# DakeQQ/Audio-Denoiser-ONNX

Measured on AMD Instinct MI355X. Metric: audio_seconds_per_second (GTCRN 16 kHz, batch=256 x 1 s chunks; RTF = 1/value), higher is better.
Workload: dtype f32; 1 GPU; GTCRN 16 kHz, batch=256 x 1 s chunks, fp32, int16 PCM in/out resident in HBM (BASELINE.json configs[1]); chunks_per_gpu=256, chunks_total=256, ranks=1, chunk_samples=16000, out_samples=15872, weights=seeded reference-architecture GTCRN (tests/golden/gtcrn_seed0.adew), stitch_all_gather=False

## Files before the change

### audio_denoiser_onnx_amd/csrc/ade_device.h

```cpp
#pragma once

#include "ade_internal.h"

namespace ade {
namespace dev {

__device__ __forceinline__ float fast_rcp(float x) { return __builtin_amdgcn_rcpf(x); }
__device__ __forceinline__ float fast_sqrt(float x) { return __builtin_amdgcn_sqrtf(x); }
__device__ __forceinline__ float fast_rsq(float x) { return __builtin_amdgcn_rsqf(x); }
__device__ __forceinline__ float sigmoid_f(float x) { return fast_rcp(1.0f + __expf(-x)); }
__device__ __forceinline__ float tanh_f(float x) {
    return 1.0f - 2.0f * fast_rcp(__expf(2.0f * x) + 1.0f);
}
__device__ __forceinline__ float prelu_f(float x, float a) { return x >= 0.0f ? x : a * x; }
__device__ __forceinline__ double shfl_xor_f64(double v, int mask) {
    union { double d; int i[2]; } u;
    u.d = v;
    u.i[0] = __shfl_xor(u.i[0], mask, 64);
    u.i[1] = __shfl_xor(u.i[1], mask, 64);
    return u.d;
}
__device__ __forceinline__ float prelu_sel(float a) { return a <= 1.0f ? __builtin_inff() : -__builtin_inff(); }
__device__ __forceinline__ float prelu_m(float x, float ax, float sel) { return __builtin_amdgcn_fmed3f(x, ax, sel); }

// ... 98 lines not shown
#define ADE_OPAQUE_V(x) asm volatile("" : "+v"(x))
#else
#define ADE_OPAQUE_V(x) ((void)0)
#endif
template <class T>
__device__ __forceinline__ T cload(const void ADE_CONSTANT_AS* p) {
    static_assert(sizeof(T) % 4 == 0, "dword-sized structs only");
    union U { T v; unsigned w[sizeof(T) / 4]; __device__ U() {} } u;
    const unsigned ADE_CONSTANT_AS* s = (const unsigned ADE_CONSTANT_AS*)p;
#pragma unroll
    for (size_t i = 0; i < sizeof(T) / 4; ++i) u.w[i] = s[i];
    return u.v;
}
typedef const float ADE_CONSTANT_AS* cfptr;
__device__ __forceinline__ cfptr cptr(const float* p) { return (cfptr)p; }

__device__ __forceinline__ void wave_sync() { __builtin_amdgcn_wave_barrier(); }
__device__ __forceinline__ float2 fcmul(float2 a, float2 b) { return make_float2(a.x * b.x - a.y * b.y, a.x * b.y + a.y * b.x); }
__device__ __forceinline__ void fradix4(float2* v) {
    const float2 a0 = make_float2(v[0].x + v[2].x, v[0].y + v[2].y);
    const float2 a1 = make_float2(v[0].x - v[2].x, v[0].y - v[2].y);
    const float2 a2 = make_float2(v[1].x + v[3].x, v[1].y + v[3].y);
    const float2 d = make_float2(v[1].x - v[3].x, v[1].y - v[3].y);
    const float2 a3 = make_float2(d.y, -d.x);
    v[0] = make_float2(a0.x + a2.x, a0.y + a2.y);
    v[1] = make_float2(a1.x + a3.x, a1.y + a3.y);
    v[2] = make_float2(a0.x - a2.x, a0.y - a2.y);
    v[3] = make_float2(a1.x - a3.x, a1.y - a3.y);
}
__device__ __forceinline__ void fft256_inplace(float2* v, float2* buf, int lane, const float2* __restrict__ tw256) {
// ... 29 lines not shown
}

#if defined(__AMDGCN__)
typedef unsigned ade_v4u __attribute__((ext_vector_type(4)));
__device__ __forceinline__ float4 xld4(const float* base, int float_off) {
    const __amdgpu_buffer_rsrc_t r = __builtin_amdgcn_make_buffer_rsrc(const_cast<float*>(base), 0, 0x7fffffff, 0x00020000);
    const ade_v4u v = __builtin_amdgcn_raw_buffer_load_b128(r, float_off * 4, 0, 16);
    return make_float4(__int_as_float((int)v.x), __int_as_float((int)v.y), __int_as_float((int)v.z), __int_as_float((int)v.w));
}
__device__ __forceinline__ void xst4(float* base, int float_off, const float4& v) {
    const __amdgpu_buffer_rsrc_t r = __builtin_amdgcn_make_buffer_rsrc(base, 0, 0x7fffffff, 0x00020000);
    ade_v4u u;
    u.x = (unsigned)__float_as_int(v.x); u.y = (unsigned)__float_as_int(v.y); u.z = (unsigned)__float_as_int(v.z); u.w = (unsigned)__float_as_int(v.w);
    __builtin_amdgcn_raw_buffer_store_b128(u, r, float_off * 4, 0, 16);
}
__device__ __forceinline__ float xld1(const float* p) { return __hip_atomic_load(p, __ATOMIC_RELAXED, __HIP_MEMORY_SCOPE_AGENT); }
__device__ __forceinline__ void xst1(float* p, float v) { __hip_atomic_store(p, v, __ATOMIC_RELAXED, __HIP_MEMORY_SCOPE_AGENT); }
__device__ __forceinline__ unsigned xflag_load(const unsigned* p) { return __hip_atomic_load(p, __ATOMIC_RELAXED, __HIP_MEMORY_SCOPE_AGENT); }
__device__ __forceinline__ void xflag_store(unsigned* p, unsigned v) { __hip_atomic_store(p, v, __ATOMIC_RELAXED, __HIP_MEMORY_SCOPE_AGENT); }
__device__ __forceinline__ void xdrain() { asm volatile("s_waitcnt vmcnt(0)" ::: "memory"); }
#else
__device__ __forceinline__ float4 xld4(const float* base, int float_off) { return *reinterpret_cast<const float4*>(base + float_off); }
__device__ __forceinline__ void xst4(float* base, int float_off, const float4& v) { *reinterpret_cast<float4*>(base + float_off) = v; }
__device__ __forceinline__ float xld1(const float* p) { return *p; }
__device__ __forceinline__ void xst1(float* p, float v) { *p = v; }
__device__ __forceinline__ unsigned xflag_load(const unsigned* p) { return *(const volatile unsigned*)p; }
__device__ __forceinline__ void xflag_store(unsigned* p, unsigned v) { *(volatile unsigned*)p = v; }
__device__ __forceinline__ void xdrain() {}
#endif
#if defined(__AMDGCN__)
__device__ __forceinline__ int xlimit() {
    const int ADE_CONSTANT_AS* p = (const int ADE_CONSTANT_AS*)__builtin_amdgcn_kernarg_segment_ptr();
    asm volatile("" : "+s"(p));
    return *p;
}
#else
__device__ __forceinline__ int xlimit() { return 20000000; }
#endif
__device__ __forceinline__ int xcode(int flag_index) { return (int)((blockIdx.x + 1u) << 4) | flag_index; }
__device__ __forceinline__ void xwait(unsigned* flag, int* err, int code) {
    if (xflag_load(flag) == 0u) {
        const long long t0 = wall_clock64();
        const int limit = xlimit();
        bool looked = false;
        do {
            __builtin_amdgcn_s_sleep(4);
            const long long dt = wall_clock64() - t0;
            if (dt > (limit >> 4) && !looked) {
                looked = true;
                if (*reinterpret_cast<volatile int*>(err) != 0) return;
            }
            if (dt > limit) {
                volatile int* const e = reinterpret_cast<volatile int*>(err);
                if (*e == 0) *e = code;
                return;
            }
        } while (xflag_load(flag) == 0u);
    }
    xflag_store(flag, 0u);
}

#if defined(__AMDGCN__)
__device__ __forceinline__ unsigned sys_load(const unsigned* p) { return __hip_atomic_load(p, __ATOMIC_RELAXED, __HIP_MEMORY_SCOPE_SYSTEM); }
__device__ __forceinline__ void sys_store(unsigned* p, unsigned v) { __hip_atomic_store(p, v, __ATOMIC_RELAXED, __HIP_MEMORY_SCOPE_SYSTEM); }
__device__ __forceinline__ void sys_acquire() { __builtin_amdgcn_fence(__ATOMIC_ACQUIRE, ""); }
__device__ __forceinline__ void sys_release() { __builtin_amdgcn_fence(__ATOMIC_RELEASE, ""); asm volatile("s_waitcnt vmcnt(0)" ::: "memory"); }
#else
__device__ __forceinline__ unsigned sys_load(const unsigned* p) { return *(const volatile unsigned*)p; }
__device__ __forceinline__ void sys_store(unsigned* p, unsigned v) { *(volatile unsigned*)p = v; }
__device__ __forceinline__ void sys_acquire() {}
__device__ __forceinline__ void sys_release() {}
#endif
__device__ __forceinline__ void wait_rows_in(const unsigned* ready, unsigned epoch, int* err, int code) {
    if (sys_load(ready) != epoch) {
        const long long t0 = wall_clock64();
        const int limit = xlimit();
        do {
            __builtin_amdgcn_s_sleep(8);
            if (wall_clock64() - t0 > limit) {
                volatile int* const e = reinterpret_cast<volatile int*>(err);
                if (*e == 0) *e = code;
                break;
            }
        } while (sys_load(ready) != epoch);
    }
    sys_acquire();
}
__device__ __forceinline__ void signal_rows_out(unsigned* count, unsigned* done, unsigned epoch, unsigned wgs) {
    sys_release();
#if defined(__AMDGCN__)
    const unsigned old = __hip_atomic_fetch_add(count, 1u, __ATOMIC_RELAXED, __HIP_MEMORY_SCOPE_AGENT);
#else
    const unsigned old = (*count)++;
#endif
    if (old + 1u == wgs) {
        xflag_store(count, 0u);
        sys_store(done, epoch);
    }
}

__device__ __forceinline__ void set_prio(int p) {
    if (p == 0) __builtin_amdgcn_s_setprio(0);
    else if (p == 1) __builtin_amdgcn_s_setprio(1);
    else if (p == 2) __builtin_amdgcn_s_setprio(2);
    else __builtin_amdgcn_s_setprio(3);
}
// ... 6 lines not shown
```

### audio_denoiser_onnx_amd/csrc/ade_stage_frontback.h

```cpp
#pragma once
#include "ade_stage_net.h"

namespace ade {
namespace stage {

constexpr int kWbuf = 264;
constexpr size_t kTabFloats = 512 + 2 * 256 + 2 * 264;
constexpr int kBmCap = 16;
constexpr int kBsCap = 4;

__device__ __forceinline__ float2 rfft_bin(float2 zk, float2 zp, float2 w) {
    const float2 e = make_float2(0.5f * (zk.x + zp.x), 0.5f * (zk.y - zp.y));
    const float2 d = make_float2(0.5f * (zk.x - zp.x), 0.5f * (zk.y + zp.y));
    const float2 o = make_float2(d.y, -d.x);
    return make_float2(e.x + (w.x * o.x - w.y * o.y), e.y + (w.x * o.y + w.y * o.x));
}

struct LdsTabs { const float* win; const float2* tw256; const float2* tw512; };
template <class G>
__device__ __forceinline__ LdsTabs stage_tables(float* dst, const FftTabs& t, int tid) {
    constexpr int kFusedThreads = G::kThreads;
    float* win = dst;
    float* tw256 = dst + 512;
    float* tw512 = tw256 + 512;
    for (int i = tid; i < 512; i += kFusedThreads) { win[i] = t.win[i]; tw256[i] = reinterpret_cast<const float*>(t.tw256)[i]; }
    for (int i = tid; i < 514; i += kFusedThreads) tw512[i] = reinterpret_cast<const float*>(t.tw512)[i];
    return LdsTabs{win, reinterpret_cast<const float2*>(tw256), reinterpret_cast<const float2*>(tw512)};
}

__device__ __forceinline__ void load_frame_pairs(const int16_t* __restrict__ row, int L, int t, int lane, bool live, bool pair_ok, int* raw, int centre = kNfft / 2) {
#pragma unroll
    for (int r = 0; r < 4; ++r) {
        const int n = lane + 64 * r;
        const int j0 = kHop * t + 2 * n - centre;
        if (!live) {
            raw[r] = 0;
        } else if (pair_ok && j0 >= 0 && j0 + 1 < L) {
            raw[r] = *reinterpret_cast<const int*>(row + j0);
        } else {
            int ja = j0, jb = j0 + 1;
            ja = ja < 0 ? -ja : (ja >= L ? 2 * (L - 1) - ja : ja);
            jb = jb < 0 ? -jb : (jb >= L ? 2 * (L - 1) - jb : jb);
            raw[r] = ((int)row[ja] & 0xffff) | ((int)row[jb] << 16);
// ... 33 lines not shown
    static_assert(kFusedThreads == 1024 || kFusedThreads == 512 || kFusedThreads == 256, "front / back conv rounds: 64 lanes per frame");
    constexpr int kBmRows = G::kLean ? 0 : kBmCap;
    const int T = sg.T, tbeg = sg.t0, tend = sg.t0 + sg.nT;
    float2* wbuf_all = reinterpret_cast<float2*>(smem);
    float* feat = smem + kTileF * kWbuf * 2;
    float4* E0 = reinterpret_cast<float4*>(feat + kFrontFeatFloats);
    float* E0f = reinterpret_cast<float*>(E0);
    float* tabmem = reinterpret_cast<float*>(E0 + 4 * kTileP1);
    float* erbw = tabmem + kTabFloats;
    float* w0t = erbw + kBmRows * kErbBands;
    float* w1t = w0t + kC0TailW;
    int* red = reinterpret_cast<int*>(w1t + kC1TailW);
    int tid_ = threadIdx.x;
    ADE_OPAQUE_V(tid_);
    const int tid = tid_, wave = tid >> 6, lane = tid & 63;
    const int16_t* row = pcm + (size_t)chunk * L;
    const int P0 = T * kF1, P = T * kFw;
    float* e0c = e0 + (size_t)chunk * kCh * P0;
    float* e1c = e1 + (size_t)chunk * kCh * P;
    float* specc = spec + (size_t)chunk * T * 2 * kBinsPad;
    ADE_CLK(32);
    const bool pair_ok = ((L & 1) == 0) && ((reinterpret_cast<size_t>(row) & 3) == 0);
    int raw[4];
    const int centre = sg.stream ? 0 : kNfft / 2;
    load_frame_pairs(row, L, tbeg + wave, lane, tbeg + wave < tend, pair_ok, raw, centre);
    const LdsTabs lt = stage_tables<G>(tabmem, tabs, tid);
    const bool erb_lds = erb.count <= kBmRows;
    if (erb_lds)
        for (int i = tid; i < erb.count * kErbBands; i += kFusedThreads) erbw[i] = erb.w[i];
    const int erb_s0 = erb.start[lane];
    for (int i = tid; i < kC0TailW; i += kFusedThreads) w0t[i] = c0.w[i];
    for (int i = tid; i < kC1TailW; i += kFusedThreads) w1t[i] = c1.w[i];
    const float b0t = c0.b[tid & 15], b1t = c1.b[tid & 15];

    if (!dc_rows) {
        int s = 0;
        if (((L & 7) == 0) && ((reinterpret_cast<size_t>(row) & 15) == 0)) {
            constexpr int kMeanLoads = 2048 / kFusedThreads;
            const int4* r4 = reinterpret_cast<const int4*>(row);
            const int4* z4 = reinterpret_cast<const int4*>(g_zero4);
            const int n4 = L >> 3;
            for (int i0 = tid; i0 < n4; i0 += kMeanLoads * kFusedThreads) {
                int4 q[kMeanLoads];
#pragma unroll
                for (int u = 0; u < kMeanLoads; ++u) {
                    const int i = i0 + u * kFusedThreads;
                    q[u] = *(i < n4 ? r4 + i : z4);
                }
#pragma unroll
                for (int u = 0; u < kMeanLoads; ++u)
                    s += (int)(short)(q[u].x & 0xffff) + (q[u].x >> 16) + (int)(short)(q[u].y & 0xffff) + (q[u].y >> 16)
                       + (int)(short)(q[u].z & 0xffff) + (q[u].z >> 16) + (int)(short)(q[u].w & 0xffff) + (q[u].w >> 16);
            }
        } else {
            for (int i = tid; i < L; i += kFusedThreads) s += (int)row[i];
        }
#pragma unroll
        for (int off = 32; off >= 1; off >>= 1) s += __shfl_xor(s, off);
        if (lane == 0) red[wave] = s;
    }
    __syncthreads();
    float dc;
    if (dc_rows) {
        dc = dc_rows[chunk];
    } else {
        long long tot = 0;
#pragma unroll
        for (int i = 0; i < kTileF; ++i) tot += red[i];
        dc = (float)((double)tot / ((double)L * 32768.0));
    }
    ADE_CLK(33);
    long long clk_prev = ADE_CLK_START();
    const cfptr c0b = cptr(c0.b), c1b = cptr(c1.b);
    const cfptr c0e = cptr(c0.w) + 5 * 9 * 16;

    for (int t0 = tbeg; t0 < tend; t0 += kTileF) {
        const int nf = tend - t0 < kTileF ? tend - t0 : kTileF;
        {
            int tq = tid;
// ... 44 lines not shown
                float* fr = feat + (size_t)wave * 3 * kErb;
#pragma unroll
                for (int r = 0; r < 5; ++r) {
                    if (r == 4 && lane != 0) break;
                    const int k = r < 4 ? lane + 64 * r : 256;
                    const float2 x = buf[k];
                    specc[((size_t)t * 2 + 0) * kBinsPad + k] = x.x;
                    specc[((size_t)t * 2 + 1) * kBinsPad + k] = x.y;
                    if (k < kErbLow) {
                        fr[k] = fast_sqrt((x.x * x.x + x.y * x.y) + 1e-12f);
                        fr[kErb + k] = x.x;
                        fr[2 * kErb + k] = x.y;
                    }
                }
                if (erb_lds) erb_merge(erbw, erb.count, erb_s0, buf, lane, fr);
                else erb_merge(erb.w, erb.count, erb_s0, buf, lane, fr);
            }
        }
        __syncthreads();
        ADE_CLK(34);
        ADE_CLK_ACC(40);
        {
            int tq = tid;
            ADE_OPAQUE_V(tq);
            const int tl = tq >> 6, g = (tq >> 4) & 3, j = tq & 15;
            if (tl < nf) {
                const float* fr = feat + (size_t)tl * 3 * kErb;
                float wa[6];
#pragma unroll
                for (int kk = 0; kk < 6; ++kk) wa[kk] = c0e[((kk >> 1) * 8 + 4 * (kk & 1) + g) * 16 + j];
                v4f cb;
// ... 124 lines not shown
    constexpr int kGroupShift = (kFusedThreads == 1024 ? 9 : (kFusedThreads == 512 ? 8 : 7));
    constexpr bool kLean = G::kLean;
    const int T = sg.T, tbeg = sg.t0, tend = sg.t0 + sg.nT;
    float4* S = reinterpret_cast<float4*>(smem);
    float* Sf = smem;
    float2* wbuf_all = reinterpret_cast<float2*>(smem);
    float4* D = S + 4 * kTileP;
    float* Df = reinterpret_cast<float*>(D);
    float* M = reinterpret_cast<float*>(D + 4 * kTileP1);
    float* acc = Df;
    float* cbuf = M + kTileF * 2 * kErbPad;
    float* tabmem = cbuf + kHop;
    float* bsw = tabmem + kTabFloats;
    float* w3t = bsw + kBsCap * kErbHigh;
    float* w4t = w3t + kC3TailW;
    float* wsum = kLean ? const_cast<float*>(tabs.win_sum) : w4t + kC4TailW;
    int* bss = reinterpret_cast<int*>(wsum + kHop);
    float* pend = kLean ? sg.xo + kXPendOff : reinterpret_cast<float*>(bss + kErbHigh);
    int tid_ = threadIdx.x;
    ADE_OPAQUE_V(tid_);
    const int tid = tid_;
    const int P0 = T * kF1, P = T * kFw;
    const float* xc = x + (size_t)chunk * kCh * P;
    const float* e1c = e1 + (size_t)chunk * kCh * P;
    const float* e0c = e0 + (size_t)chunk * kCh * P0;
    const float* specc = spec + (size_t)chunk * T * 2 * kBinsPad;
    const int trim = sg.stream ? 0 : kHop;
    const int out_len = sg.stream ? kHop * T : kHop * (T - 1);
    int16_t* po = pcm ? pcm + (size_t)chunk * out_len : nullptr;
    float* fo32 = f32 ? f32 + (size_t)chunk * out_len : nullptr;
    ADE_CLK(48);

    auto issue_s = [&](int t0n, bool go, float4* sa, float4* sb) {
        const int nfn = tend - t0n < kTileF ? tend - t0n : kTileF;
        int tq = tid;
        ADE_OPAQUE_V(tq);
        const bool on = go && tq < kSThreads;
#pragma unroll
        for (int i = 0; i < 3; ++i) {
            const int u = tq + kSThreads * i, q = u / kTileP, idx = u - q * kTileP;
            const int idc = idx < nfn * kFw ? idx : 0;
            const size_t off = ((size_t)q * P + (size_t)t0n * kFw + idc) * 4;
            sa[i] = on ? *reinterpret_cast<const float4*>(xc + off) : make_float4(0.0f, 0.0f, 0.0f, 0.0f);
            sb[i] = on ? *reinterpret_cast<const float4*>(e1c + off) : make_float4(0.0f, 0.0f, 0.0f, 0.0f);
        }
// ... 13 lines not shown
        ADE_OPAQUE_V(tq);
        const int g = tq >> kGroupShift, tl = (tq >> 5) & (kTileF - 1), m = tq & 31;
        const bool on = go && tl < nfn;
        const int pe = on ? tl * kF1 + 2 * m : 0;
#pragma unroll
        for (int h = 0; h < 2; ++h) {
            const float* src = e0c + ((size_t)(2 * g + h) * P0 + (size_t)t0n * kF1 + pe) * 4;
            ea[h] = on ? *reinterpret_cast<const float4*>(src) : make_float4(0.0f, 0.0f, 0.0f, 0.0f);
            eb[h] = on ? *reinterpret_cast<const float4*>(src + 4) : make_float4(0.0f, 0.0f, 0.0f, 0.0f);
        }
    };
    float4 sa0[3], sb0[3];
    issue_s(tbeg, true, sa0, sb0);
    float4 ea[2], eb[2];
    issue_e0(tbeg, true, ea, eb);
    const LdsTabs lt = stage_tables<G>(tabmem, tabs, tid);
    if (!kLean)
        for (int i = tid; i < kHop; i += kFusedThreads) wsum[i] = tabs.win_sum[i];
    const bool bs_lds = bs.count <= kBsCap;
    int bs_s[4] = {0, 0, 0, 0};
    if (bs_lds) {
        for (int i = tid; i < bs.count * kErbHigh; i += kFusedThreads) bsw[i] = bs.w[i];
        if (!kLean) {
            for (int i = tid; i < kErbHigh; i += kFusedThreads) bss[i] = bs.start[i];
        } else {
            int tq = tid;
            ADE_OPAQUE_V(tq);
            const int lane = tq & 63;
#pragma unroll
            for (int r = 1; r < 5; ++r) {
                const int k = r < 4 ? lane + 64 * r : 256;
                bs_s[r - 1] = (k >= kErbLow && (r < 4 || lane == 0)) ? bs.start[k - kErbLow] : 0;
            }
        }
    }
    for (int i = tid; i < kC3TailW; i += kFusedThreads) w3t[i] = c3.w[(i < 128 ? 2 : 4) * 128 + (i & 127)];
    for (int i = tid; i < kC4TailW; i += kFusedThreads) w4t[i] = c4.w[(i < 32 ? 2 : 4) * 32 + (i & 31)];
    const float b3t = c3.b[tid & 15], b4t = c4.b[tid & 1];
    for (int i = tid; i < kHop; i += kFusedThreads) cbuf[i] = 0.0f;
    const cfptr c3b = cptr(c3.b), c4b = cptr(c4.b), c4w = cptr(c4.w);
    commit_s(sa0, sb0);
    long long clk_prev = ADE_CLK_START();

    for (int t0 = tbeg; t0 < tend; t0 += kTileF) {
        const int nf = tend - t0 < kTileF ? tend - t0 : kTileF;
        float sre[5], sim[5];
        float wsr[4] = {1.0f, 1.0f, 1.0f, 1.0f};
        if (kLean) ld4(wsum + ((tid * 4) & (kHop - 1)), wsr);
        {
            int tq = tid;
            ADE_OPAQUE_V(tq);
            const int wave = tq >> 6, lane = tq & 63;
            const int tcp = wave < nf ? t0 + wave : t0;
// ... 134 lines not shown
                if (k < kErbLow) {
                    m0 = mr[k];
                    m1 = mr[kErbPad + k];
                } else {
                    const int o = k - kErbLow;
                    m0 = 0.0f; m1 = 0.0f;
                    if (bs_lds) {
                        const int s0 = kLean ? bs_s[r > 0 ? r - 1 : 0] : bss[o];
                        for (int n = 0; n < bs.count; ++n) {
                            const float wv = bsw[n * kErbHigh + o];
                            const int jj = min(s0 + n, kErbBands - 1);
                            m0 += mr[kErbLow + jj] * wv;
                            m1 += mr[kErbPad + kErbLow + jj] * wv;
                        }
                    } else {
                        const int s0 = bs.start[o];
                        for (int n = 0; n < bs.count; ++n) {
                            const float wv = bs.w[n * kErbHigh + o];
                            const int jj = min(s0 + n, kErbBands - 1);
                            m0 += mr[kErbLow + jj] * wv;
                            m1 += mr[kErbPad + kErbLow + jj] * wv;
                        }
                    }
                }
                float2 y = make_float2(__fmaf_rn(xr, m0, -(xi * m1)), __fmaf_rn(xi, m0, xr * m1));
                if (k == 0 || k == 256) y.y = 0.0f;
                buf[k] = y;
            }
            wave_sync();
            float2 v[4];
#pragma unroll
            for (int r = 0; r < 4; ++r) {
                const int k = lane + 64 * r;
// ... 106 lines not shown
```

### audio_denoiser_onnx_amd/csrc/ade_stage_net.h

```cpp
#pragma once
#include "ade_device.h"

#include <type_traits>

#ifndef ADE_DP_INTER_MFMA
#define ADE_DP_INTER_MFMA 0
#endif

namespace ade {
namespace stage {

using namespace dev;


template <int NT, int TMAX, int WAVES_PER_SIMD>
struct Geo {
    static constexpr int kThreads = NT;
    static constexpr int kWavesPerSimd = WAVES_PER_SIMD;
    static constexpr int kTmax = TMAX;
    static constexpr int kPmax = TMAX * kFw;
    static constexpr int kPosPerThread = (kPmax + NT - 1) / NT;
    static constexpr int kTileF = NT / 64;
    static constexpr int kProdBase = ((TMAX * (kFw / 3) + 63) / 64) * 64;
    static constexpr bool kLean = NT < 512;
// ... 34 lines not shown
                                              bool next_full = false) {
    constexpr int kFusedThreads = G::kThreads, kTmaxFused = G::kTmax, kPmax = G::kPmax, kPosPerThread = G::kPosPerThread;
    float4* H = smem;
    float* zt = reinterpret_cast<float*>(smem + 4 * kPmax);
    float* at = zt + kTmaxFused * 8;
    float* GI = reinterpret_cast<float*>(smem + 2 * kPmax);
    float* HS = GI + kTmaxFused * 48;
    const int T = sg.nT;
    const int P = T * kFw;
    const int Ps = sg.T * kFw;
    int tid_ = threadIdx.x;
    if (kFusedThreads == 512 && sg.swap) tid_ ^= (tid_ & 256) >> 1;
    ADE_OPAQUE_V(tid_);
    const int tid = tid_;
    const size_t cbase = (size_t)chunk * kCh * Ps + (size_t)sg.t0 * kFw * 4;
    const float* ac = a + cbase;
    const float* sc = skip ? skip + cbase : nullptr;
    float* oc = out + cbase;
    const cfptr c_pw1_b = cptr(w.pw1_b), c_dw_b = cptr(w.dw_b), c_pw2_b = cptr(w.pw2_b);
    cfptr c_pw1, c_dw, c_pw2;
    ADE_SCALAR_COPY(c_pw1, cptr(w.pw1));
    ADE_SCALAR_COPY(c_dw, cptr(w.dw));
    ADE_SCALAR_COPY(c_pw2, cptr(w.pw2));
    const float pw1_slope = w.pw1_slope, dw_slope = w.dw_slope;
    const float pw1_sel = prelu_sel(pw1_slope), dw_sel = prelu_sel(dw_slope);
    const int dilation = w.dilation;
    ADE_CLK(0);

    if (!x1_in_lds) {
        constexpr int kIt = (kPmax + kFusedThreads - 1) / kFusedThreads;
        float x[kIt][8], y[kIt][8];
#pragma unroll
        for (int i = 0; i < kIt; ++i) {
// ... 169 lines not shown
    ADE_CLK(2);
#pragma unroll
    for (int pr = 0; pr < kPairs; ++pr) {
        const int it = 2 * pr + (g >> 1);
        const int pu = (it * kWaves + wave) * 16 + jn;
        if (it < kTiles && pu < P) H[(g & 1) * kPmax + pu] = h1r[pr];
    }
    __syncthreads();
    ADE_CLK(3);

    v2f wr_raw[8];
    float bh_raw = 0.0f;
    {
        const int j = tid & 15, row = (tid >> 4) & 3;
        const int gsel = (row & 1) ? 2 : (row >> 1);
        const float* pk = w.gru + j * 78 + 24 + gsel * 16;
#pragma unroll
        for (int m = 0; m < 8; ++m) wr_raw[m] = tid < 64 ? mk2(pk[2 * m], pk[2 * m + 1]) : mk2(0.0f, 0.0f);
        if (tid < 64) bh_raw = w.gru[j * 78 + 75 + gsel];
    }
    const float* nsc = (next_x1 && next_skip) ? next_skip + cbase : nullptr;
    float nsk[kPosPerThread][8];
    auto request_next_skip = [&]() {
#pragma unroll
        for (int i = 0; i < kPosPerThread; ++i) {
            const int p = tid + i * kFusedThreads;
            if (nsc && p < P) {
                pl_ld8(nsc, Ps, p, 0, nsk[i]);
            } else {
#pragma unroll
                for (int k = 0; k < 8; ++k) nsk[i][k] = 0.0f;
            }
        }
    };
    request_next_skip();
    {
// ... 6 lines not shown
                const int f = j + 16 * u;
                if (f < kFw) {
                    const float4 a0 = H[t * kFw + f], a1 = H[kPmax + t * kFw + f];
                    e[0] += a0.x * a0.x; e[1] += a0.y * a0.y; e[2] += a0.z * a0.z; e[3] += a0.w * a0.w;
                    e[4] += a1.x * a1.x; e[5] += a1.y * a1.y; e[6] += a1.z * a1.z; e[7] += a1.w * a1.w;
                }
            }
#pragma unroll
            for (int c = 0; c < 8; ++c) {
                e[c] += row_ror<8>(e[c]);
                e[c] += row_ror<4>(e[c]);
                e[c] += row_ror<2>(e[c]);
                e[c] += row_ror<1>(e[c]);
                e[c] = e[c] * (1.0f / (float)kFw);
            }
            const float* pk = w.gru + j * 78;
#pragma unroll
            for (int g = 0; g < 3; ++g) {
                float sacc = pk[72 + g];
#pragma unroll
                for (int k = 0; k < 8; ++k) sacc += pk[g * 8 + k] * e[k];
                if (tr < T) GI[t * 48 + g * 16 + j] = sacc * (g == 2 ? 2.0f * kLog2e : -kLog2e);
            }
        }
    }
    if (sg.prev && tid == 0) xwait(sg.fi + kXFlagTra + blk, sg.err, xcode(kXFlagTra + blk));
    __syncthreads();
    ADE_CLK(4);
    ADE_CLK(5);
    if (tid >= 64) {
        constexpr int kLanes = kFusedThreads - 64, kIt = (kPmax + kLanes - 1) / kLanes;
// ... 63 lines not shown
            *hsp = hc;
            hsp += hs_step;
            gi = gnx;
        }
        set_prio(sg.base_prio);
        if (sg.next) {
            if (row == 3) xst1(sg.xo + kXTraOff + blk * 16 + j, hv);
            xdrain();
            if (tid == 48) xflag_store(sg.fo + kXFlagTra + blk, 1u);
        }
    }
    __syncthreads();
    ADE_CLK(6);
    for (int idx = tid; idx < T * 8; idx += kFusedThreads) {
        const int t = idx >> 3, c = idx & 7;
        const float* fr = w.fc + c * 17;
        float s = fr[16];
#pragma unroll
        for (int k = 0; k < 16; ++k) s += fr[k] * HS[t * 16 + k];
        at[idx] = sigmoid_f(s);
    }
    __syncthreads();
    ADE_CLK(7);
#pragma unroll
    for (int pr = 0; pr < kPairs; ++pr) {
        const int it = 2 * pr + (g >> 1);
        const int pu = (it * kWaves + wave) * 16 + jn;
        if (it < kTiles && pu < P) {
            const float4 gt = *reinterpret_cast<const float4*>(at + (pu / kFw) * 8 + 4 * (g & 1));
            H[(2 + (g & 1)) * kPmax + pu] = make_float4(h1r[pr].x * gt.x, h1r[pr].y * gt.y, h1r[pr].z * gt.z, h1r[pr].w * gt.w);
        }
// ... 166 lines not shown
            lnw[u] = gw[ic];
            lnb[u] = gb[ic];
        }
    };
    auto ln_tab_st = [&]() {
#pragma unroll
        for (int u = 0; u < kLnPerLane; ++u) {
            const int i = tid + u * kFusedThreads;
            if (i < kFw * kCh) {
                lnt[i] = lnw[u];
                lnt[kFw * kCh + i] = lnb[u];
            }
        }
    };
    const size_t cbase = (size_t)chunk * kCh * Ps + (size_t)sg.t0 * kFw * 4;
    const float* xc = x + cbase;
    float* oc = out + cbase;

    LnRes rx;
    ln_tab_ld(w.intra_ln_w, w.intra_ln_b);
    const FcW fwB = fc_w_ld(w.intra_fc, w.intra_fc_b, tid);
    float gw0, gw1, gwh, gb6[6];
    {
        const int wave = __builtin_amdgcn_readfirstlane(tid >> 6), g = (tid >> 4) & 3, j = tid & 15, c = j & 3;
        const int grp = (wave >> 1) & 1, dir = wave & 1;
        const float* pk = w.intra_gru + (grp * 8 + dir * 4 + (j >> 2)) * 42;
        const int gi = c == 3 ? 2 : c;
        gw0 = pk[gi * 8 + g];
        gw1 = pk[gi * 8 + 4 + g];
        gwh = pk[24 + (c == 3 ? 0 : c) * 4 + g];
        const float* pb = w.intra_gru + (grp * 8 + dir * 4 + g) * 42;
#pragma unroll
        for (int k = 0; k < 6; ++k) gb6[k] = pb[36 + k];
    }
    ln_tab_st();
    ADE_CLK(16);
    {
        constexpr float kS = -kLog2e, kN = 2.0f * kLog2e;
        if (!x_in_lds) {
            float4 v[kPosPerThread][4];
#pragma unroll
            for (int i = 0; i < kPosPerThread; ++i) {
                const int p = tid + i * kFusedThreads, pc = p < P ? p : P - 1;
#pragma unroll
                for (int q = 0; q < 4; ++q) v[i][q] = *reinterpret_cast<const float4*>(xc + ((size_t)q * Ps + pc) * 4);
            }
// ... 50 lines not shown
            }
            set_prio(sg.base_prio);
            ln_res_ld(Rf, kPmax, ln_row(tid, T), rx);
            __syncthreads();
            float* const hw = Rf + ((size_t)(grp * 2 + DIR) * kPmax + tc * kFw) * 4 + g;
            if (live) {
#pragma unroll
                for (int s = 0; s < kFw; ++s) hw[(DIR ? kFw - 1 - s : s) * 4] = hout[s];
            }
        };
        if (dir) run(std::integral_constant<int, 1>{});
        else run(std::integral_constant<int, 0>{});
    }
    __syncthreads();
    ADE_CLK(17);
    ln_tab_ld(w.inter_ln_w, w.inter_ln_b);
    fc_ln_rows<G>(R, fwB, lnt, lnt + kFw * kCh, T, P, tid, rx,
        [&](int p, const float (&m)[16]) {
#pragma unroll
            for (int q = 0; q < 4; ++q) R[q * kPmax + p] = make_float4(m[4 * q], m[4 * q + 1], m[4 * q + 2], m[4 * q + 3]);
            pl_st16(oc, Ps, p, m);
        },
        [&](int p, int c, float m) {
            Rf[((size_t)(c >> 2) * kPmax + p) * 4 + (c & 3)] = m;
            oc[((size_t)(c >> 2) * Ps + p) * 4 + (c & 3)] = m;
        });
    if (sg.prev && tid == 0) xwait(sg.fi + kXFlagInter + blk, sg.err, xcode(kXFlagInter + blk));
    __syncthreads();
    ln_tab_st();
    ADE_CLK(18);
#if ADE_DP_INTER_MFMA
    {
        constexpr float kS = -kLog2e, kN = 2.0f * kLog2e;
        constexpr int kWaves = kFusedThreads / 64, kTilesC = 6;
        static_assert(kWaves % 2 == 0, "a wavefront's tiles share its group");
        const int wave = __builtin_amdgcn_readfirstlane(tid >> 6);
        const int g = (tid >> 4) & 3, j = tid & 15;
        const int grp = wave & 1;
        float ax[2][2], ah[2][2];
        v4f cb[2];
#pragma unroll
        for (int U = 0; U < 2; ++U) {
            const int c = j & 3;
            const float* pk = w.inter_gru + (grp * 8 + 4 * U + (j >> 2)) * 54;
            const float sc_ = c < 2 ? kS : kN;
            const int gi = c == 3 ? 2 : c;
#pragma unroll
            for (int kk = 0; kk < 2; ++kk) {
                ax[U][kk] = c == 2 ? 0.0f : pk[gi * 8 + 4 * kk + g] * sc_;
                ah[U][kk] = c == 3 ? 0.0f : pk[24 + c * 8 + 4 * kk + g] * sc_;
            }
            const float* pb = w.inter_gru + (grp * 8 + 4 * U + g) * 54;
            cb[U][0] = (pb[48] + pb[51]) * kS;
            cb[U][1] = (pb[49] + pb[52]) * kS;
            cb[U][2] = pb[53] * kN;
            cb[U][3] = pb[50] * kN;
        }
        auto run = [&](auto nt_c) {
            constexpr int NT = decltype(nt_c)::value;
            float h[NT][2];
            bool live[NT];
            float* xp[NT];
            float* xs[NT];
            v4f dx[NT][2];
#pragma unroll
            for (int c = 0; c < NT; ++c) {
                const int tile = wave + c * kWaves, f = (tile >> 1) * 16 + j;
// ... 51 lines not shown
                    }
                }
                xdrain();
            }
        };
        const int nt = wave < kTilesC ? (kTilesC - 1 - wave) / kWaves + 1 : 0;
        static_assert((kTilesC + kWaves - 1) / kWaves <= 2, "at most two tiles per wavefront");
        if (nt == 2) run(std::integral_constant<int, 2>{});
        else if (nt == 1) run(std::integral_constant<int, 1>{});
    }
#else
    {
        constexpr int kRows = G::kThreads / 16;
        const int row = tid >> 4, q = tid & 15;
        const int grp = q & 1, unit = q >> 1;
        const float* pk = w.inter_gru + (grp * 8 + unit) * 54;
        int ks[8];
        ks[0] = unit;
#define ADE_KS(S) ks[S] = ((int)row_ror<2 * S>((float)q)) >> 1;
        ADE_KS(1) ADE_KS(2) ADE_KS(3) ADE_KS(4) ADE_KS(5) ADE_KS(6) ADE_KS(7)
#undef ADE_KS
        constexpr float kS = -kLog2e, kN = 2.0f * kLog2e;
        v2f wi_rz[8], wh_rz[8], wi_n[4], wh_n[4];
#pragma unroll
        for (int k = 0; k < 8; ++k) {
            wi_rz[k] = mk2(pk[k] * kS, pk[8 + k] * kS);
            wh_rz[k] = mk2(pk[24 + ks[k]] * kS, pk[32 + ks[k]] * kS);
        }
#pragma unroll
        for (int m = 0; m < 4; ++m) {
            wi_n[m] = mk2(pk[16 + 2 * m] * kN, pk[16 + 2 * m + 1] * kN);
// ... 56 lines not shown
                    if (live[c]) xst1(sg.xo + kXInterOff + blk * (kFw * 16) + fc_[c] * 16 + q, h[c]);
                xdrain();
            }
        };
        const int row0 = (tid >> 6) * 4, nc = row0 < kFw ? (kFw - 1 - row0) / kRows + 1 : 0;
        static_assert((kFw + kRows - 1) / kRows <= 3, "at most three columns per 16-lane row");
        if (nc == 3) run(std::integral_constant<int, 3>{});
        else if (nc == 2) run(std::integral_constant<int, 2>{});
        else if (nc == 1) run(std::integral_constant<int, 1>{});
    }
#endif
    __syncthreads();
    if (sg.next && tid == 0) xflag_store(sg.fo + kXFlagInter + blk, 1u);
    ADE_CLK(19);
    {
        const float* nsc = (next_x1 && next_skip) ? next_skip + cbase : nullptr;
        const FcW fwD = fc_w_ld(w.inter_fc, w.inter_fc_b, tid);
        LnRes rm;
        ln_res_ld(oc, Ps, ln_row(tid, T), rm);
        fc_ln_rows<G>(R, fwD, lnt, lnt + kFw * kCh, T, P, tid, rm,
            [&](int p, const float (&o)[16]) {
                if (store_lo) {
                    pl_st16(oc, Ps, p, o);
                } else {
                    st4(oc + ((size_t)2 * Ps + p) * 4, o + 8);
                    st4(oc + ((size_t)3 * Ps + p) * 4, o + 12);
                }
                if (next_full) {
#pragma unroll
                    for (int q = 0; q < 4; ++q) R[q * kPmax + p] = make_float4(o[4 * q], o[4 * q + 1], o[4 * q + 2], o[4 * q + 3]);
                }
                if (next_x1) {
// ... 22 lines not shown
```

Before: 781,600 audio-s/s.

## Use global address space pointers and batch table staging through registers

Casts device pointers to the global address space (address_space(1)) so the compiler can emit global_load/store instead of flat memory ops, including for the atomics used in cross-workgroup flags. It also restructures the LDS table and weight staging in the front and back stages: all global loads are issued into registers first, then written to LDS, so load latency overlaps instead of running as serialized copy loops. The cost is higher register pressure during the prologue, which could reduce occupancy.

Measured after the change: 793,200 audio-s/s (median of 6 runs). 1.5% higher.

```diff
diff --git a/audio_denoiser_onnx_amd/csrc/ade_device.h b/audio_denoiser_onnx_amd/csrc/ade_device.h
--- a/audio_denoiser_onnx_amd/csrc/ade_device.h
+++ b/audio_denoiser_onnx_amd/csrc/ade_device.h
@@ -136,6 +136,33 @@
 }
 typedef const float ADE_CONSTANT_AS* cfptr;
 __device__ __forceinline__ cfptr cptr(const float* p) { return (cfptr)p; }
+
+#if defined(__has_attribute)
+#if __has_attribute(address_space)
+#define ADE_GLOBAL_AS __attribute__((address_space(1)))
+#endif
+#endif
+#ifndef ADE_GLOBAL_AS
+#define ADE_GLOBAL_AS
+#endif
+template <class T> __device__ __forceinline__ T* gptr(T* p) {
+#if defined(__AMDGCN__)
+    T ADE_GLOBAL_AS* q = (T ADE_GLOBAL_AS*)p;
+    asm("" : "+s"(q));
+    return (T*)q;
+#else
+    return p;
+#endif
+}
+template <class T> __device__ __forceinline__ T* gptr_lane(T* p) {
+#if defined(__AMDGCN__)
+    T ADE_GLOBAL_AS* q = (T ADE_GLOBAL_AS*)p;
+    asm("" : "+v"(q));
+    return (T*)q;
+#else
+    return p;
+#endif
+}
 
 __device__ __forceinline__ void wave_sync() { __builtin_amdgcn_wave_barrier(); }
 __device__ __forceinline__ float2 fcmul(float2 a, float2 b) { return make_float2(a.x * b.x - a.y * b.y, a.x * b.y + a.y * b.x); }
@@ -195,10 +222,12 @@
     u.x = (unsigned)__float_as_int(v.x); u.y = (unsigned)__float_as_int(v.y); u.z = (unsigned)__float_as_int(v.z); u.w = (unsigned)__float_as_int(v.w);
     __builtin_amdgcn_raw_buffer_store_b128(u, r, float_off * 4, 0, 16);
 }
-__device__ __forceinline__ float xld1(const float* p) { return __hip_atomic_load(p, __ATOMIC_RELAXED, __HIP_MEMORY_SCOPE_AGENT); }
-__device__ __forceinline__ void xst1(float* p, float v) { __hip_atomic_store(p, v, __ATOMIC_RELAXED, __HIP_MEMORY_SCOPE_AGENT); }
-__device__ __forceinline__ unsigned xflag_load(const unsigned* p) { return __hip_atomic_load(p, __ATOMIC_RELAXED, __HIP_MEMORY_SCOPE_AGENT); }
-__device__ __forceinline__ void xflag_store(unsigned* p, unsigned v) { __hip_atomic_store(p, v, __ATOMIC_RELAXED, __HIP_MEMORY_SCOPE_AGENT); }
+__device__ __forceinline__ float xld1(const float* p) { return __hip_atomic_load(gptr_lane(p), __ATOMIC_RELAXED, __HIP_MEMORY_SCOPE_AGENT); }
+__device__ __forceinline__ void xst1(float* p, float v) { __hip_atomic_store(gptr_lane(p), v, __ATOMIC_RELAXED, __HIP_MEMORY_SCOPE_AGENT); }
+__device__ __forceinline__ unsigned xflag_load(const unsigned* p) { return __hip_atomic_load(gptr_lane(p), __ATOMIC_RELAXED, __HIP_MEMORY_SCOPE_AGENT); }
+__device__ __forceinline__ void xflag_store(unsigned* p, unsigned v) { __hip_atomic_store(gptr_lane(p), v, __ATOMIC_RELAXED, __HIP_MEMORY_SCOPE_AGENT); }
+__device__ __forceinline__ int xerr_load(const int* p) { return __hip_atomic_load(gptr_lane(p), __ATOMIC_RELAXED, __HIP_MEMORY_SCOPE_SYSTEM); }
+__device__ __forceinline__ void xerr_store(int* p, int v) { __hip_atomic_store(gptr_lane(p), v, __ATOMIC_RELAXED, __HIP_MEMORY_SCOPE_SYSTEM); }
 __device__ __forceinline__ void xdrain() { asm volatile("s_waitcnt vmcnt(0)" ::: "memory"); }
 #else
 __device__ __forceinline__ float4 xld4(const float* base, int float_off) { return *reinterpret_cast<const float4*>(base + float_off); }
@@ -207,6 +236,8 @@
 __device__ __forceinline__ void xst1(float* p, float v) { *p = v; }
 __device__ __forceinline__ unsigned xflag_load(const unsigned* p) { return *(const volatile unsigned*)p; }
 __device__ __forceinline__ void xflag_store(unsigned* p, unsigned v) { *(volatile unsigned*)p = v; }
+__device__ __forceinline__ int xerr_load(const int* p) { return *(const volatile int*)p; }
+__device__ __forceinline__ void xerr_store(int* p, int v) { *(volatile int*)p = v; }
 __device__ __forceinline__ void xdrain() {}
 #endif
 #if defined(__AMDGCN__)
@@ -229,11 +260,10 @@
             const long long dt = wall_clock64() - t0;
             if (dt > (limit >> 4) && !looked) {
                 looked = true;
-                if (*reinterpret_cast<volatile int*>(err) != 0) return;
+                if (xerr_load(err) != 0) return;
             }
             if (dt > limit) {
-                volatile int* const e = reinterpret_cast<volatile int*>(err);
-                if (*e == 0) *e = code;
+                if (xerr_load(err) == 0) xerr_store(err, code);
                 return;
             }
         } while (xflag_load(flag) == 0u);
@@ -242,8 +272,8 @@
 }
 
 #if defined(__AMDGCN__)
-__device__ __forceinline__ unsigned sys_load(const unsigned* p) { return __hip_atomic_load(p, __ATOMIC_RELAXED, __HIP_MEMORY_SCOPE_SYSTEM); }
-__device__ __forceinline__ void sys_store(unsigned* p, unsigned v) { __hip_atomic_store(p, v, __ATOMIC_RELAXED, __HIP_MEMORY_SCOPE_SYSTEM); }
+__device__ __forceinline__ unsigned sys_load(const unsigned* p) { return __hip_atomic_load(gptr_lane(p), __ATOMIC_RELAXED, __HIP_MEMORY_SCOPE_SYSTEM); }
+__device__ __forceinline__ void sys_store(unsigned* p, unsigned v) { __hip_atomic_store(gptr_lane(p), v, __ATOMIC_RELAXED, __HIP_MEMORY_SCOPE_SYSTEM); }
 __device__ __forceinline__ void sys_acquire() { __builtin_amdgcn_fence(__ATOMIC_ACQUIRE, ""); }
 __device__ __forceinline__ void sys_release() { __builtin_amdgcn_fence(__ATOMIC_RELEASE, ""); asm volatile("s_waitcnt vmcnt(0)" ::: "memory"); }
 #else
@@ -259,8 +289,7 @@
         do {
             __builtin_amdgcn_s_sleep(8);
             if (wall_clock64() - t0 > limit) {
-                volatile int* const e = reinterpret_cast<volatile int*>(err);
-                if (*e == 0) *e = code;
+                if (xerr_load(err) == 0) xerr_store(err, code);
                 break;
             }
         } while (sys_load(ready) != epoch);
@@ -270,7 +299,7 @@
 __device__ __forceinline__ void signal_rows_out(unsigned* count, unsigned* done, unsigned epoch, unsigned wgs) {
     sys_release();
 #if defined(__AMDGCN__)
-    const unsigned old = __hip_atomic_fetch_add(count, 1u, __ATOMIC_RELAXED, __HIP_MEMORY_SCOPE_AGENT);
+    const unsigned old = __hip_atomic_fetch_add(gptr_lane(count), 1u, __ATOMIC_RELAXED, __HIP_MEMORY_SCOPE_AGENT);
 #else
     const unsigned old = (*count)++;
 #endif
diff --git a/audio_denoiser_onnx_amd/csrc/ade_stage_frontback.h b/audio_denoiser_onnx_amd/csrc/ade_stage_frontback.h
--- a/audio_denoiser_onnx_amd/csrc/ade_stage_frontback.h
+++ b/audio_denoiser_onnx_amd/csrc/ade_stage_frontback.h
@@ -17,16 +17,63 @@
 }
 
 struct LdsTabs { const float* win; const float2* tw256; const float2* tw512; };
+template <int N, int NT> constexpr int per_lane() { return (N + NT - 1) / NT; }
 template <class G>
-__device__ __forceinline__ LdsTabs stage_tables(float* dst, const FftTabs& t, int tid) {
-    constexpr int kFusedThreads = G::kThreads;
-    float* win = dst;
-    float* tw256 = dst + 512;
-    float* tw512 = tw256 + 512;
-    for (int i = tid; i < 512; i += kFusedThreads) { win[i] = t.win[i]; tw256[i] = reinterpret_cast<const float*>(t.tw256)[i]; }
-    for (int i = tid; i < 514; i += kFusedThreads) tw512[i] = reinterpret_cast<const float*>(t.tw512)[i];
-    return LdsTabs{win, reinterpret_cast<const float2*>(tw256), reinterpret_cast<const float2*>(tw512)};
-}
+struct TabRegs {
+    static constexpr int kNT = G::kThreads, kN = per_lane<512, kNT>(), kM = per_lane<514, kNT>();
+    float win[kN], t256[kN], t512[kM];
+    __device__ __forceinline__ void ld(const FftTabs& t, int tid) {
+        const float* const gwin = gptr(t.win);
+        const float* const g256 = gptr(reinterpret_cast<const float*>(t.tw256));
+        const float* const g512 = gptr(reinterpret_cast<const float*>(t.tw512));
+#pragma unroll
+        for (int u = 0; u < kN; ++u) {
+            const int i = tid + u * kNT, ic = i < 512 ? i : 511;
+            win[u] = gwin[ic];
+            t256[u] = g256[ic];
+        }
+#pragma unroll
+        for (int u = 0; u < kM; ++u) {
+            const int i = tid + u * kNT;
+            t512[u] = g512[i < 514 ? i : 513];
+        }
+    }
+    __device__ __forceinline__ LdsTabs st(float* dst, int tid) const {
+        float* w = dst;
+        float* a = dst + 512;
+        float* b = a + 512;
+#pragma unroll
+        for (int u = 0; u < kN; ++u) {
+            const int i = tid + u * kNT;
+            if (i < 512) { w[i] = win[u]; a[i] = t256[u]; }
+        }
+#pragma unroll
+        for (int u = 0; u < kM; ++u) {
+            const int i = tid + u * kNT;
+            if (i < 514) b[i] = t512[u];
+        }
+        return LdsTabs{w, reinterpret_cast<const float2*>(a), reinterpret_cast<const float2*>(b)};
+    }
+};
+template <int N, int NT>
+struct CopyRegs {
+    static constexpr int kU = per_lane<N, NT>() > 0 ? per_lane<N, NT>() : 1;
+    float v[kU];
+    __device__ __forceinline__ void ld(const float* src, int n, int tid) {
+#pragma unroll
+        for (int u = 0; u < kU; ++u) {
+            const int i = tid + u * NT;
+            v[u] = src[i < n ? i : 0];
+        }
+    }
+    __device__ __forceinline__ void st(float* dst, int n, int tid) const {
+#pragma unroll
+        for (int u = 0; u < kU; ++u) {
+            const int i = tid + u * NT;
+            if (i < n) dst[i] = v[u];
+        }
+    }
+};
 
 __device__ __forceinline__ void load_frame_pairs(const int16_t* __restrict__ row, int L, int t, int lane, bool live, bool pair_ok, int* raw, int centre = kNfft / 2) {
 #pragma unroll
@@ -90,24 +137,33 @@
     int tid_ = threadIdx.x;
     ADE_OPAQUE_V(tid_);
     const int tid = tid_, wave = tid >> 6, lane = tid & 63;
-    const int16_t* row = pcm + (size_t)chunk * L;
+    const int16_t* row = gptr(pcm) + (size_t)chunk * L;
     const int P0 = T * kF1, P = T * kFw;
-    float* e0c = e0 + (size_t)chunk * kCh * P0;
-    float* e1c = e1 + (size_t)chunk * kCh * P;
-    float* specc = spec + (size_t)chunk * T * 2 * kBinsPad;
+    float* e0c = gptr(e0) + (size_t)chunk * kCh * P0;
+    float* e1c = gptr(e1) + (size_t)chunk * kCh * P;
+    float* specc = gptr(spec) + (size_t)chunk * T * 2 * kBinsPad;
+    const float* const erb_w = gptr(erb.w);
     ADE_CLK(32);
     const bool pair_ok = ((L & 1) == 0) && ((reinterpret_cast<size_t>(row) & 3) == 0);
     int raw[4];
     const int centre = sg.stream ? 0 : kNfft / 2;
     load_frame_pairs(row, L, tbeg + wave, lane, tbeg + wave < tend, pair_ok, raw, centre);
-    const LdsTabs lt = stage_tables<G>(tabmem, tabs, tid);
     const bool erb_lds = erb.count <= kBmRows;
-    if (erb_lds)
-        for (int i = tid; i < erb.count * kErbBands; i += kFusedThreads) erbw[i] = erb.w[i];
-    const int erb_s0 = erb.start[lane];
-    for (int i = tid; i < kC0TailW; i += kFusedThreads) w0t[i] = c0.w[i];
-    for (int i = tid; i < kC1TailW; i += kFusedThreads) w1t[i] = c1.w[i];
-    const float b0t = c0.b[tid & 15], b1t = c1.b[tid & 15];
+    const int erb_n = erb_lds ? erb.count * kErbBands : 0;
+    TabRegs<G> tr;
+    CopyRegs<kBmRows * kErbBands, kFusedThreads> er;
+    CopyRegs<kC0TailW, kFusedThreads> w0r;
+    CopyRegs<kC1TailW, kFusedThreads> w1r;
+    tr.ld(tabs, tid);
+    if (kBmRows > 0) er.ld(erb_w, erb_n, tid);
+    const int erb_s0 = gptr(erb.start)[lane];
+    w0r.ld(gptr(c0.w), kC0TailW, tid);
+    w1r.ld(gptr(c1.w), kC1TailW, tid);
+    const float b0t = gptr(c0.b)[tid & 15], b1t = gptr(c1.b)[tid & 15];
+    const LdsTabs lt = tr.st(tabmem, tid);
+    if (kBmRows > 0) er.st(erbw, erb_n, tid);
+    w0r.st(w0t, kC0TailW, tid);
+    w1r.st(w1t, kC1TailW, tid);
 
     if (!dc_rows) {
         int s = 0;
@@ -138,7 +194,7 @@
     __syncthreads();
     float dc;
     if (dc_rows) {
-        dc = dc_rows[chunk];
+        dc = gptr(dc_rows)[chunk];
     } else {
         long long tot = 0;
 #pragma unroll
@@ -213,7 +269,7 @@
                     }
                 }
                 if (erb_lds) erb_merge(erbw, erb.count, erb_s0, buf, lane, fr);
-                else erb_merge(erb.w, erb.count, erb_s0, buf, lane, fr);
+                else erb_merge(erb_w, erb.count, erb_s0, buf, lane, fr);
             }
         }
         __syncthreads();
@@ -368,21 +424,23 @@
     float* bsw = tabmem + kTabFloats;
     float* w3t = bsw + kBsCap * kErbHigh;
     float* w4t = w3t + kC3TailW;
-    float* wsum = kLean ? const_cast<float*>(tabs.win_sum) : w4t + kC4TailW;
+    float* wsum = kLean ? const_cast<float*>(gptr(tabs.win_sum)) : w4t + kC4TailW;
     int* bss = reinterpret_cast<int*>(wsum + kHop);
-    float* pend = kLean ? sg.xo + kXPendOff : reinterpret_cast<float*>(bss + kErbHigh);
+    float* pend = kLean ? gptr(sg.xo) + kXPendOff : reinterpret_cast<float*>(bss + kErbHigh);
     int tid_ = threadIdx.x;
     ADE_OPAQUE_V(tid_);
     const int tid = tid_;
     const int P0 = T * kF1, P = T * kFw;
-    const float* xc = x + (size_t)chunk * kCh * P;
-    const float* e1c = e1 + (size_t)chunk * kCh * P;
-    const float* e0c = e0 + (size_t)chunk * kCh * P0;
-    const float* specc = spec + (size_t)chunk * T * 2 * kBinsPad;
+    const float* xc = gptr(x) + (size_t)chunk * kCh * P;
+    const float* e1c = gptr(e1) + (size_t)chunk * kCh * P;
+    const float* e0c = gptr(e0) + (size_t)chunk * kCh * P0;
+    const float* specc = gptr(spec) + (size_t)chunk * T * 2 * kBinsPad;
+    const float* const bs_w = gptr(bs.w);
+    const int* const bs_start = gptr(bs.start);
     const int trim = sg.stream ? 0 : kHop;
     const int out_len = sg.stream ? kHop * T : kHop * (T - 1);
-    int16_t* po = pcm ? pcm + (size_t)chunk * out_len : nullptr;
-    float* fo32 = f32 ? f32 + (size_t)chunk * out_len : nullptr;
+    int16_t* po = pcm ? gptr(pcm) + (size_t)chunk * out_len : nullptr;
+    float* fo32 = f32 ? gptr(f32) + (size_t)chunk * out_len : nullptr;
     ADE_CLK(48);
 
     auto issue_s = [&](int t0n, bool go, float4* sa, float4* sb) {
@@ -426,29 +484,40 @@
     issue_s(tbeg, true, sa0, sb0);
     float4 ea[2], eb[2];
     issue_e0(tbeg, true, ea, eb);
-    const LdsTabs lt = stage_tables<G>(tabmem, tabs, tid);
-    if (!kLean)
-        for (int i = tid; i < kHop; i += kFusedThreads) wsum[i] = tabs.win_sum[i];
     const bool bs_lds = bs.count <= kBsCap;
+    const int bs_n = bs_lds ? bs.count * kErbHigh : 0;
+    TabRegs<G> tr;
+    CopyRegs<kHop, kFusedThreads> wsr0;
+    CopyRegs<kBsCap * kErbHigh, kFusedThreads> bsr;
+    tr.ld(tabs, tid);
+    if (!kLean) wsr0.ld(gptr(tabs.win_sum), kHop, tid);
+    bsr.ld(bs_w, bs_n, tid);
     int bs_s[4] = {0, 0, 0, 0};
-    if (bs_lds) {
-        for (int i = tid; i < bs.count * kErbHigh; i += kFusedThreads) bsw[i] = bs.w[i];
-        if (!kLean) {
-            for (int i = tid; i < kErbHigh; i += kFusedThreads) bss[i] = bs.start[i];
-        } else {
-            int tq = tid;
-            ADE_OPAQUE_V(tq);
-            const int lane = tq & 63;
-#pragma unroll
-            for (int r = 1; r < 5; ++r) {
-                const int k = r < 4 ? lane + 64 * r : 256;
-                bs_s[r - 1] = (k >= kErbLow && (r < 4 || lane == 0)) ? bs.start[k - kErbLow] : 0;
-            }
-        }
-    }
-    for (int i = tid; i < kC3TailW; i += kFusedThreads) w3t[i] = c3.w[(i < 128 ? 2 : 4) * 128 + (i & 127)];
-    for (int i = tid; i < kC4TailW; i += kFusedThreads) w4t[i] = c4.w[(i < 32 ? 2 : 4) * 32 + (i & 31)];
-    const float b3t = c3.b[tid & 15], b4t = c4.b[tid & 1];
+    int bss_r = 0;
+    if (!kLean) {
+        static_assert(kLean || kErbHigh <= kFusedThreads, "one ERB-split start index per lane");
+        bss_r = bs_start[tid < kErbHigh ? tid : 0];
+    } else {
+        int tq = tid;
+        ADE_OPAQUE_V(tq);
+        const int lane = tq & 63;
+#pragma unroll
+        for (int r = 1; r < 5; ++r) {
+            const int k = r < 4 ? lane + 64 * r : 256;
+            const int v = bs_start[(k >= kErbLow && (r < 4 || lane == 0)) ? k - kErbLow : 0];
+            bs_s[r - 1] = (bs_lds && k >= kErbLow && (r < 4 || lane == 0)) ? v : 0;
+        }
+    }
+    static_assert(kC3TailW <= kFusedThreads && kC4TailW <= kFusedThreads, "one tail weight of each deconvolution per lane");
+    const float w3r = gptr(c3.w)[((tid & 255) < 128 ? 2 : 4) * 128 + (tid & 127)];
+    const float w4r = gptr(c4.w)[((tid & 63) < 32 ? 2 : 4) * 32 + (tid & 31)];
+    const float b3t = gptr(c3.b)[tid & 15], b4t = gptr(c4.b)[tid & 1];
+    const LdsTabs lt = tr.st(tabmem, tid);
+    if (!kLean) wsr0.st(wsum, kHop, tid);
+    bsr.st(bsw, bs_n, tid);
+    if (!kLean && bs_lds && tid < kErbHigh) bss[tid] = bss_r;
+    if (tid < kC3TailW) w3t[tid] = w3r;
+    if (tid < kC4TailW) w4t[tid] = w4r;
     for (int i = tid; i < kHop; i += kFusedThreads) cbuf[i] = 0.0f;
     const cfptr c3b = cptr(c3.b), c4b = cptr(c4.b), c4w = cptr(c4.w);
     commit_s(sa0, sb0);
@@ -613,9 +682,9 @@
                             m1 += mr[kErbPad + kErbLow + jj] * wv;
                         }
                     } else {
-                        const int s0 = bs.start[o];
+                        const int s0 = bs_start[o];
                         for (int n = 0; n < bs.count; ++n) {
-                            const float wv = bs.w[n * kErbHigh + o];
+                            const float wv = bs_w[n * kErbHigh + o];
                             const int jj = min(s0 + n, kErbBands - 1);
                             m0 += mr[kErbLow + jj] * wv;
                             m1 += mr[kErbPad + kErbLow + jj] * wv;
diff --git a/audio_denoiser_onnx_amd/csrc/ade_stage_net.h b/audio_denoiser_onnx_amd/csrc/ade_stage_net.h
--- a/audio_denoiser_onnx_amd/csrc/ade_stage_net.h
+++ b/audio_denoiser_onnx_amd/csrc/ade_stage_net.h
@@ -72,9 +72,10 @@
     ADE_OPAQUE_V(tid_);
     const int tid = tid_;
     const size_t cbase = (size_t)chunk * kCh * Ps + (size_t)sg.t0 * kFw * 4;
-    const float* ac = a + cbase;
-    const float* sc = skip ? skip + cbase : nullptr;
-    float* oc = out + cbase;
+    const float* ac = gptr(a) + cbase;
+    const float* sc = skip ? gptr(skip) + cbase : nullptr;
+    float* oc = gptr(out) + cbase;
+    const float* const w_gru = gptr(w.gru);
     const cfptr c_pw1_b = cptr(w.pw1_b), c_dw_b = cptr(w.dw_b), c_pw2_b = cptr(w.pw2_b);
     cfptr c_pw1, c_dw, c_pw2;
     ADE_SCALAR_COPY(c_pw1, cptr(w.pw1));
@@ -274,12 +275,12 @@
     {
         const int j = tid & 15, row = (tid >> 4) & 3;
         const int gsel = (row & 1) ? 2 : (row >> 1);
-        const float* pk = w.gru + j * 78 + 24 + gsel * 16;
+        const float* pk = w_gru + j * 78 + 24 + gsel * 16;
 #pragma unroll
         for (int m = 0; m < 8; ++m) wr_raw[m] = tid < 64 ? mk2(pk[2 * m], pk[2 * m + 1]) : mk2(0.0f, 0.0f);
-        if (tid < 64) bh_raw = w.gru[j * 78 + 75 + gsel];
-    }
-    const float* nsc = (next_x1 && next_skip) ? next_skip + cbase : nullptr;
+        if (tid < 64) bh_raw = w_gru[j * 78 + 75 + gsel];
+    }
+    const float* nsc = (next_x1 && next_skip) ? gptr(next_skip) + cbase : nullptr;
     float nsk[kPosPerThread][8];
     auto request_next_skip = [&]() {
 #pragma unroll
@@ -316,7 +317,7 @@
                 e[c] += row_ror<1>(e[c]);
                 e[c] = e[c] * (1.0f / (float)kFw);
             }
-            const float* pk = w.gru + j * 78;
+            const float* pk = w_gru + j * 78;
 #pragma unroll
             for (int g = 0; g < 3; ++g) {
                 float sacc = pk[72 + g];
@@ -410,7 +411,7 @@
     ADE_CLK(6);
     for (int idx = tid; idx < T * 8; idx += kFusedThreads) {
         const int t = idx >> 3, c = idx & 7;
-        const float* fr = w.fc + c * 17;
+        const float* fr = gptr(w.fc) + c * 17;
         float s = fr[16];
 #pragma unroll
         for (int k = 0; k < 16; ++k) s += fr[k] * HS[t * 16 + k];
@@ -607,22 +608,22 @@
         }
     };
     const size_t cbase = (size_t)chunk * kCh * Ps + (size_t)sg.t0 * kFw * 4;
-    const float* xc = x + cbase;
-    float* oc = out + cbase;
+    const float* xc = gptr(x) + cbase;
+    float* oc = gptr(out) + cbase;
 
     LnRes rx;
-    ln_tab_ld(w.intra_ln_w, w.intra_ln_b);
-    const FcW fwB = fc_w_ld(w.intra_fc, w.intra_fc_b, tid);
+    ln_tab_ld(gptr(w.intra_ln_w), gptr(w.intra_ln_b));
+    const FcW fwB = fc_w_ld(gptr(w.intra_fc), gptr(w.intra_fc_b), tid);
     float gw0, gw1, gwh, gb6[6];
     {
         const int wave = __builtin_amdgcn_readfirstlane(tid >> 6), g = (tid >> 4) & 3, j = tid & 15, c = j & 3;
         const int grp = (wave >> 1) & 1, dir = wave & 1;
-        const float* pk = w.intra_gru + (grp * 8 + dir * 4 + (j >> 2)) * 42;
+        const float* pk = gptr(w.intra_gru) + (grp * 8 + dir * 4 + (j >> 2)) * 42;
         const int gi = c == 3 ? 2 : c;
         gw0 = pk[gi * 8 + g];
         gw1 = pk[gi * 8 + 4 + g];
         gwh = pk[24 + (c == 3 ? 0 : c) * 4 + g];
-        const float* pb = w.intra_gru + (grp * 8 + dir * 4 + g) * 42;
+        const float* pb = gptr(w.intra_gru) + (grp * 8 + dir * 4 + g) * 42;
 #pragma unroll
         for (int k = 0; k < 6; ++k) gb6[k] = pb[36 + k];
     }
@@ -703,7 +704,7 @@
     }
     __syncthreads();
     ADE_CLK(17);
-    ln_tab_ld(w.inter_ln_w, w.inter_ln_b);
+    ln_tab_ld(gptr(w.inter_ln_w), gptr(w.inter_ln_b));
     fc_ln_rows<G>(R, fwB, lnt, lnt + kFw * kCh, T, P, tid, rx,
         [&](int p, const float (&m)[16]) {
 #pragma unroll
@@ -731,7 +732,7 @@
 #pragma unroll
         for (int U = 0; U < 2; ++U) {
             const int c = j & 3;
-            const float* pk = w.inter_gru + (grp * 8 + 4 * U + (j >> 2)) * 54;
+            const float* pk = gptr(w.inter_gru) + (grp * 8 + 4 * U + (j >> 2)) * 54;
             const float sc_ = c < 2 ? kS : kN;
             const int gi = c == 3 ? 2 : c;
 #pragma unroll
@@ -739,7 +740,7 @@
                 ax[U][kk] = c == 2 ? 0.0f : pk[gi * 8 + 4 * kk + g] * sc_;
                 ah[U][kk] = c == 3 ? 0.0f : pk[24 + c * 8 + 4 * kk + g] * sc_;
             }
-            const float* pb = w.inter_gru + (grp * 8 + 4 * U + g) * 54;
+            const float* pb = gptr(w.inter_gru) + (grp * 8 + 4 * U + g) * 54;
             cb[U][0] = (pb[48] + pb[51]) * kS;
             cb[U][1] = (pb[49] + pb[52]) * kS;
             cb[U][2] = pb[53] * kN;
@@ -821,7 +822,7 @@
         constexpr int kRows = G::kThreads / 16;
         const int row = tid >> 4, q = tid & 15;
         const int grp = q & 1, unit = q >> 1;
-        const float* pk = w.inter_gru + (grp * 8 + unit) * 54;
+        const float* pk = gptr(w.inter_gru) + (grp * 8 + unit) * 54;
         int ks[8];
         ks[0] = unit;
 #define ADE_KS(S) ks[S] = ((int)row_ror<2 * S>((float)q)) >> 1;
@@ -908,8 +909,8 @@
     if (sg.next && tid == 0) xflag_store(sg.fo + kXFlagInter + blk, 1u);
     ADE_CLK(19);
     {
-        const float* nsc = (next_x1 && next_skip) ? next_skip + cbase : nullptr;
-        const FcW fwD = fc_w_ld(w.inter_fc, w.inter_fc_b, tid);
+        const float* nsc = (next_x1 && next_skip) ? gptr(next_skip) + cbase : nullptr;
+        const FcW fwD = fc_w_ld(gptr(w.inter_fc), gptr(w.inter_fc_b), tid);
         LnRes rm;
         ln_res_ld(oc, Ps, ln_row(tid, T), rm);
         fc_ln_rows<G>(R, fwD, lnt, lnt + kFw * kCh, T, P, tid, rm,
```
